# nickmccleery/open-kinematics

Measured on AMD Instinct MI355X. Metric: constraint solves/sec (sweep steps/sec), double-wishbone bump sweep, higher is better.
Workload: dtype f64

## Files before the change

### __graft_entry__.py

```python

from __future__ import annotations

import os
import sys

REPO = os.path.dirname(os.path.abspath(__file__))
if REPO not in sys.path:
    sys.path.insert(0, REPO)


def build() -> None:
    os.environ.setdefault("PYTORCH_ROCM_ARCH", "gfx950")
    from open_kinematics_amd import _lib

    path = _lib.build()
    if not os.path.exists(path):
        raise RuntimeError("libokx.so was not produced")
    from oracle import oracle as oracle_mod

    oracle_mod.build()
    import open_kinematics_amd

    lib = _lib.load()
    missing = [name for name in _lib.EXPORTS + _lib.DEBUG_EXPORTS if not hasattr(lib, name)]
# ... 8 lines not shown

def precompile_baseline_kernels() -> None:
    from open_kinematics_amd import _lib
    from open_kinematics_amd._abi import HostProgram
    from open_kinematics_amd.workloads import axle_grid_problem, bump_sweep_problem, macpherson_grid_problem

    lib = _lib.load()
    programs = []
    evaluated = []
    for make in (bump_sweep_problem, lambda n, line_mode: macpherson_grid_problem(n, n, line_mode),
                 lambda n, line_mode: axle_grid_problem(n, n, line_mode)):
        for mode in ("pinned", "softnorm"):
            programs.append(make(4, line_mode=mode)[0])
    from open_kinematics_amd.input import load_geometry, load_sweep
    from open_kinematics_amd.metrics import corner_roles
    from open_kinematics_amd.solver import dropin_program
    from open_kinematics_amd.sweep import sweep_program
    from open_kinematics_amd.workloads import geometry_path

    for geometry, sweeps in (("geometry.yaml", ("bump_sweep.yaml", "sweep.yaml")),
                             ("axle_geometry_rocker.yaml", ("axle_rocker_sweep.yaml",)),
                             ("axle_geometry.yaml", ("axle_sweep.yaml",)),
                             ("axle_geometry_explicit.yaml", ("axle_sweep.yaml",)),
                             ("macpherson_axle_geometry.yaml", ("axle_sweep.yaml",)),
                             ("corner_rocker_geometry.yaml", ("sweep.yaml",)),
                             ("corner_strut_geometry.yaml", ("sweep.yaml",)),
                             ("corner_strut_rocker_geometry.yaml", ("sweep.yaml",))):
        suspension = load_geometry(geometry_path(geometry))
        for sweep_file in sweeps:
            sweep = load_sweep(geometry_path(sweep_file), suspension)
            programs.append(dropin_program(suspension.initial_state(), suspension.constraints(), sweep,
                                           suspension.derived_spec())[0])
            programs.append(sweep_program(suspension, sweep)[0])
            if not hasattr(suspension, "corners"):
                evaluated += [(p, corner_roles(suspension, p)) for p in programs[-2:]]
            else:
                evaluated += _axle_evaluated(suspension, programs[-2:])
    evaluated.append((bump_sweep_problem(4)[0], corner_roles(load_geometry(geometry_path("geometry.yaml")), bump_sweep_problem(4)[0])))
    evaluated.append((macpherson_grid_problem(4, 4)[0],
                      corner_roles(load_geometry(geometry_path("macpherson_geometry.yaml")), macpherson_grid_problem(4, 4)[0])))
    evaluated += _axle_evaluated(load_geometry(geometry_path("axle_geometry_rocker.yaml")), [axle_grid_problem(4, 4)[0]])
    import glob

    import numpy as np

    from open_kinematics_amd.program import ConstraintProgram

    golden = os.path.join(os.path.dirname(os.path.abspath(__file__)), "tests", "golden")
    for path in sorted(glob.glob(os.path.join(golden, "[ctue]*.npz"))):
        arrays = dict(np.load(path, allow_pickle=False))
        if "prog_point_kind" not in arrays and not any(k.startswith("prog_") for k in arrays):
            continue
        fixture = ConstraintProgram.from_arrays(arrays, prefix="prog_")
        programs += [fixture.with_line_mode("pinned"), fixture]
    import yaml

    from open_kinematics_amd.input import build_suspension, build_sweep

    for path in sorted(glob.glob(os.path.join(golden, "[cte]*.npz"))):
        arrays = dict(np.load(path, allow_pickle=False))
        if "geometry_yaml" not in arrays or "sweep_yaml" not in arrays:
            continue
        try:
            suspension = build_suspension(yaml.safe_load(str(arrays["geometry_yaml"])))
            sweep = build_sweep(yaml.safe_load(str(arrays["sweep_yaml"])), suspension)
            pair = [dropin_program(suspension.initial_state(), suspension.constraints(), sweep, suspension.derived_spec())[0],
                    sweep_program(suspension, sweep)[0]]
        except Exception as error:
            print(f"precompile: drop-in programs of {os.path.basename(path)} skipped ({type(error).__name__}: {error})", file=sys.stderr)
            continue
        programs += pair
        if not hasattr(suspension, "corners"):
            evaluated += [(p, corner_roles(suspension, p)) for p in pair]
        else:
            evaluated += _axle_evaluated(suspension, pair)
    from open_kinematics_amd.metrics import roles_from_arrays

    for name in ("c1_dw_corner", "c4_macpherson_grid", "e2e_sweep"):
        arrays = dict(np.load(os.path.join(golden, f"{name}.npz"), allow_pickle=False))
        fixture = ConstraintProgram.from_arrays(arrays, prefix="prog_").with_line_mode("pinned")
        names = [fixture.point_keys[k].lower_name for k in fixture.out_point]
        metric_arrays = dict(np.load(os.path.join(golden, f"metrics_{name}.npz"), allow_pickle=False))
        evaluated.append((fixture, roles_from_arrays(names, fixture.design_pos[fixture.out_point], metric_arrays)[0]))
    from open_kinematics_amd.precompile import precompile_job

    seen, jobs = set(), []
    for program, roles in [(p, None) for p in programs] + evaluated:
        arrays = program.to_arrays()
        key = (program.line_mode, tuple((k, v.tobytes()) for k, v in sorted(arrays.items()) if k != "target_desc"),
               None if roles is None else bytes(roles))
        if key not in seen:
            seen.add(key)
            jobs.append((arrays, program.line_mode, None if roles is None else bytes(roles)))
    workers = max(1, min(6, (os.cpu_count() or 2) - 1, len(jobs)))
    try:
        results = _precompile_in_workers(jobs, workers)
    except OSError as error:
        print(f"precompile: worker pool unavailable ({type(error).__name__}: {error}); compiling sequentially", file=sys.stderr)
        results = [precompile_job(job) for job in jobs]
    for rc, message in results:
        if rc == -2:
            continue
        if rc != 0:
            raise RuntimeError(f"quad kernel precompilation failed: {message}")


def _precompile_in_workers(jobs: list, workers: int) -> list:
    import json
    import pickle
    import selectors
    import subprocess
    import tempfile

    results = [None] * len(jobs)
    pending = list(range(len(jobs)))[::-1]
    env = dict(os.environ, PYTHONPATH=os.pathsep.join([REPO] + [p for p in [os.environ.get("PYTHONPATH")] if p]))
    with tempfile.TemporaryDirectory() as tmp:
        path = os.path.join(tmp, "jobs.pkl")
        with open(path, "wb") as fh:
            pickle.dump(jobs, fh)
        procs = [subprocess.Popen([sys.executable, "-m", "open_kinematics_amd.precompile", "--jobs", path], cwd=REPO, env=env,
                                  stdin=subprocess.PIPE, stdout=subprocess.PIPE, text=True) for _ in range(workers)]
        selector = selectors.DefaultSelector()

        def feed(proc) -> bool:
            if not pending:
                proc.stdin.close()
                return False
            proc.stdin.write(f"{pending.pop()}\n")
            proc.stdin.flush()
            return True

        try:
            for proc in procs:
                if feed(proc):
                    selector.register(proc.stdout, selectors.EVENT_READ, proc)
            while selector.get_map():
                for key, _ in selector.select():
                    line = key.fileobj.readline()
                    if not line:
                        raise RuntimeError(f"a precompile worker exited with status {key.data.wait()}")
                    index, rc, message = json.loads(line)
                    results[index] = (rc, message)
                    if not feed(key.data):
                        selector.unregister(key.fileobj)
        finally:
            for proc in procs:
                if proc.poll() is None and not proc.stdin.closed:
                    proc.stdin.close()
            for proc in procs:
                proc.wait()
    return results


def _axle_evaluated(axle, programs) -> list:
    from open_kinematics_amd.metrics import axle_evaluation_roles

    out = []
    for program in programs:
        try:
            out.append((program, axle_evaluation_roles(axle, program)[0]))
        except ValueError as error:
            print(f"precompile: axle evaluated module skipped ({error})", file=sys.stderr)
    return out


def smoke() -> None:
    import numpy as np
    import torch

    from open_kinematics_amd.batch import DeviceProgram
    from open_kinematics_amd.workloads import bump_sweep_problem
    from oracle.oracle import Oracle

    if not torch.cuda.is_available():
        raise RuntimeError("smoke() needs cuda:0")
    torch.cuda.set_device(0)
    program, targets = bump_sweep_problem(101)
    dp = DeviceProgram(program, "cuda:0")
    res = dp.solve(torch.as_tensor(targets, device="cuda:0"))
    torch.cuda.synchronize()
    info = res.info()
    if not np.all((info["flags"] & 7) == 1):
        raise RuntimeError(f"smoke: not every step converged: flags={np.unique(info['flags'])}")
    orc = Oracle(program).sweep(targets, 1e-15, 1e-15, 1e-15, warm_start=False)
    err = float(np.max(np.abs(res.positions.cpu().numpy() - orc.positions)))
    if not err <= 1e-9:
        raise RuntimeError(f"smoke: device vs oracle max |dpos| = {err:.3e} mm > 1e-9")
    print(f"smoke ok: 101 steps, max|device - oracle| = {err:.2e} mm, "
          f"iterations mean {info['iterations'].mean():.2f}")


if __name__ == "__main__":
    build()
    if len(sys.argv) > 1 and sys.argv[1] == "smoke":
        smoke()
```

### open_kinematics_amd/csrc/okx_quadgen.cpp

```cpp
#include <cstdarg>
#include <cstdio>
#include <cstdlib>
#include <functional>
#include <map>
#include <set>
#include <string>
#include <vector>

#include "okx_gen.hpp"
#include "okx_plan.hpp"
#include "okx_quad.hpp"

namespace okx {
namespace {

struct LV {
  std::string n;
  int sg = 1;
};

struct Blk {
  bool scaled = true;
  std::string s;
  std::string col[3];
};

struct BlkTerm {
  Blk b;
  int sg;
};

class Gen : public GenBase {
 public:
  explicit Gen(const DevProgram& prog, const PairView* pair = nullptr)
      : GenBase(prog, pair && pair->joins.size() == 1 ? pair->couple_point : -1), pv(pair) {}

  const PairView* pv;

  static std::string sel(int i0, int i1) {
    if (i0 == i1) return std::to_string(i0);
    return "(q1 ? " + std::to_string(i1) + " : " + std::to_string(i0) + ")";
  }
  std::string point3(int p) const {
    return pv ? sel(3 * pv->pt[0][p], 3 * pv->pt[1][p]) : std::to_string(3 * p);
  }
  std::string point4(int p) const {
    return pv ? sel(4 * pv->pt[0][p], 4 * pv->pt[1][p]) : std::to_string(4 * p);
  }
  std::string crow8(int i, int k) const {
    return pv ? sel(8 * pv->row[0][i] + k, 8 * pv->row[1][i] + k) : std::to_string(8 * i + k);
  }
  std::string trow8(int i, int k) const {
    if (!pv) return std::to_string(8 * i + k);
    const int t = target_of_row(i);
    int t0 = pv->tgt[0][t], t1 = pv->tgt[1][t];
    if (t0 < 0) t0 = t1;
    if (t1 < 0) t1 = t0;
    return sel(8 * (pv->n_prog_crows + t0) + k, 8 * (pv->n_prog_crows + t1) + k);
  }
  std::string target_slot(int t) const {
    if (!pv) return std::to_string(t);
    int t0 = pv->tgt[0][t], t1 = pv->tgt[1][t];
    if (t0 < 0) t0 = t1;
    if (t1 < 0) t1 = t0;
    return sel(t0, t1);
  }
  std::string target_enable(int t) const {
    if (!pv) return "1.0";
    const bool e0 = pv->tgt[0][t] >= 0, e1 = pv->tgt[1][t] >= 0;
    if (e0 && e1) return "1.0";
    return e0 ? "(q1 ? 0.0 : 1.0)" : "(q1 ? 1.0 : 0.0)";
  }
  std::string dop_slot(int e) const { return pv ? sel(pv->dop[0][e], pv->dop[1][e]) : std::to_string(e); }
  std::map<std::string, std::string> rot1_, rot2_;
  std::map<std::string, std::vector<std::string>> bc_;
  std::map<int, std::map<int, Blk>> dblk;
  bool nz[kMaxFree][kMaxFree] = {};

  static std::string f_str(const char* fmt, ...) {
    char buf[256];
    va_list ap;
    va_start(ap, fmt);
// ... 245 lines not shown
            nb.scaled = false;
            apply_t(col, nb.col);
            acc[kv.first].push_back({nb, sg});
          }
        }
        dblk[e] = combine(acc);
      }
      return true;
    }
    why = "unknown derived op";
    return false;
  }

  struct RowOut {
    std::string r;
    std::vector<std::pair<int, LV>> partial;
    std::string absres;
  };

  std::string dp(int e) {
    auto key = std::make_pair(-1 - e, 0);
    auto it = hoisted_names.find(key);
    if (it != hoisted_names.end()) return it->second;
    char name[48], line[200];
    std::snprintf(name, sizeof(name), "hd%d", e);
    const std::string home = scalar_home(name);
    std::snprintf(line, sizeof(line), "      %s%s = a.dop_param[%s];\n", sdecl(), home.c_str(), dop_slot(e).c_str());
    hoisted += line;
    hoisted_names[key] = home;
    return home;
  }

  std::string rp(int i, int k) {
    i = pin_leader(i);
    auto key = std::make_pair(i, 100 + k);
    auto it = hoisted_names.find(key);
    if (it != hoisted_names.end()) return it->second;
    char name[48], line[200];
    std::snprintf(name, sizeof(name), "hs%d_%d", i, k);
    const std::string home = scalar_home(name);
    if (i < P.n_crows)
      std::snprintf(line, sizeof(line), "      %s%s = gq[%s];\n", sdecl(), home.c_str(), crow8(i, k).c_str());
    else
      std::snprintf(line, sizeof(line), "      %s%s = a.row_param[%s];\n", sdecl(), home.c_str(), trow8(i, k).c_str());
    hoisted += line;
    hoisted_names[key] = home;
    return home;
  }
  std::string hoisted;
  std::map<std::pair<int, int>, std::string> hoisted_names;
  bool lds_constants = false;

  int n_scalar_slots = 0, n_lane_slots = 0;
  bool scalars_in_regs = false, lanes_in_regs = false;
  std::string scalar_home(const char* name) {
    if (!lds_constants || scalars_in_regs) return name;
    return "hsl[" + std::to_string(16 * n_scalar_slots++) + " + qs]";
  }
  std::string lane_home(const char* name) {
    if (!lds_constants || lanes_in_regs) return name;
    return "hql[" + std::to_string(64 * n_lane_slots++) + " + lane]";
  }
  const char* sdecl() const { return lds_constants && !scalars_in_regs ? "" : "const double "; }
  const char* ldecl() const { return lds_constants && !lanes_in_regs ? "" : "const double "; }
  std::string rpv(int i, int k0) {
    i = pin_leader(i);
    auto key = std::make_pair(i, k0);
    auto it = hoisted_names.find(key);
    if (it != hoisted_names.end()) return it->second;
    char name[48], line[200];
    std::snprintf(name, sizeof(name), "hq%d_%d", i, k0);
    const std::string home = lane_home(name);
    if (i < P.n_crows)
      std::snprintf(line, sizeof(line), "      %s%s = ld3(gq + %s + cc, c);\n", ldecl(), home.c_str(), crow8(i, k0).c_str());
    else
      std::snprintf(line, sizeof(line), "      %s%s = ld3(a.row_param + %s + cc, c) * %s;\n", ldecl(), home.c_str(),
                    trow8(i, k0).c_str(), target_enable(target_of_row(i)).c_str());
    hoisted += line;
    hoisted_names[key] = home;
    return home;
  }
  std::map<int, std::string> pin_cross_;

  bool row(int i, RowOut* ro) {
    const int type = P.row_type[i];
    const int* pts = P.row_pts[i];
    f("    // row %d (type %d)", i, type);
    std::string r = "r" + std::to_string(i);
    ro->r = r;
    ro->absres = "fabs(" + r + ")";
    switch (type) {
      case OKX_ROW_DISTANCE:
      case OKX_ROW_SPHERICAL: {
        std::string d = vsub(pn(pts[1]), pn(pts[0]));
        std::string s = dot(d, d);
        std::string root = tmp("rt"), inv = tmp("iv"), g = tmp("g");
        f("    double %s, %s; fast_sqrt_rsqrt(%s + EPS_SQ, &%s, &%s);", root.c_str(), inv.c_str(), s.c_str(),
          root.c_str(), inv.c_str());
        f("    const double %s = %s * %s;", g.c_str(), d.c_str(), inv.c_str());
        if (type == OKX_ROW_DISTANCE)
          f("    const double %s = (%s - EPS) - %s;", r.c_str(), root.c_str(), rp(i, 0).c_str());
        else
          f("    const double %s = %s - EPS;", r.c_str(), root.c_str());
        ro->partial.push_back({pts[0], {g, -1}});
        ro->partial.push_back({pts[1], {g, 1}});
        return true;
      }
      case OKX_ROW_ANGLE:
      case OKX_ROW_THREE_POINT_ANGLE: {
        std::string v1, v2;
        if (type == OKX_ROW_ANGLE) {
          v1 = vsub(pn(pts[1]), pn(pts[0]));
          v2 = vsub(pn(pts[3]), pn(pts[2]));
        } else {
          v1 = vsub(pn(pts[0]), pn(pts[1]));
          v2 = vsub(pn(pts[2]), pn(pts[1]));
        }
        std::string cv = cross(v1, v2);
        std::string c2 = dot(cv, cv);
        std::string dt = dot(v1, v2);
        std::string s = tmp("s"), is = tmp("is"), t15 = tmp("t");
        f("    const double %s = EPS_SQ + %s;", t15.c_str(), c2.c_str());
        f("    double %s, %s; fast_sqrt_rsqrt(%s, &%s, &%s);", s.c_str(), is.c_str(), t15.c_str(), s.c_str(),
          is.c_str());
        std::string inv = tmp("iv"), ka = tmp("ka"), kb = tmp("kb");
        f("    const double %s = fast_rcp(%s + %s * %s);", inv.c_str(), t15.c_str(), dt.c_str(), dt.c_str());
        f("    const double %s = %s * %s * %s, %s = %s * %s;", ka.c_str(), dt.c_str(), inv.c_str(), is.c_str(),
          kb.c_str(), s.c_str(), inv.c_str());
        std::string w1 = cross(v2, cv), w2 = cross(cv, v1);
        std::string g1 = tmp("g"), g2 = tmp("g");
        f("    const double %s = %s * %s - %s * %s;", g1.c_str(), ka.c_str(), w1.c_str(), kb.c_str(), v2.c_str());
        f("    const double %s = %s * %s - %s * %s;", g2.c_str(), ka.c_str(), w2.c_str(), kb.c_str(), v1.c_str());
        f("    const double %s = lean_atan2_pos<%s>(%s - EPS, %s, %s) - %s;", r.c_str(), pv ? "true" : "false", s.c_str(), dt.c_str(), pv ? "atl" : "nullptr",
          rp(i, 0).c_str());
        if (type == OKX_ROW_ANGLE) {
          ro->partial.push_back({pts[0], {g1, -1}});
          ro->partial.push_back({pts[1], {g1, 1}});
          ro->partial.push_back({pts[2], {g2, -1}});
          ro->partial.push_back({pts[3], {g2, 1}});
        } else {
          std::string gm = tmp("g");
          f("    const double %s = -%s - %s;", gm.c_str(), g1.c_str(), g2.c_str());
          ro->partial.push_back({pts[0], {g1, 1}});
          ro->partial.push_back({pts[1], {gm, 1}});
          ro->partial.push_back({pts[2], {g2, 1}});
        }
        return true;
      }
      case OKX_ROW_VECTORS_PARALLEL:
      case OKX_ROW_VECTORS_PERPENDICULAR: {
        std::string v1 = vsub(pn(pts[1]), pn(pts[0])), v2 = vsub(pn(pts[3]), pn(pts[2]));
        std::string n1 = dot(v1, v1), n2 = dot(v2, v2);
        std::string s1 = tmp("s"), s2 = tmp("s"), g1 = tmp("g"), g2 = tmp("g");
        f("    const double %s = sqrt(EPS_SQ + %s), %s = sqrt(EPS_SQ + %s);", s1.c_str(), n1.c_str(), s2.c_str(), n2.c_str());
        if (type == OKX_ROW_VECTORS_PARALLEL) {
          std::string cv = cross(v1, v2);
          std::string c2 = dot(cv, cv);
          std::string sc = tmp("s");
          f("    const double %s = sqrt(EPS_SQ + %s);", sc.c_str(), c2.c_str());
          std::string w1 = cross(v2, cv), w2 = cross(cv, v1);
          std::string k26 = tmp("k"), k19 = tmp("k"), k31 = tmp("k");
          f("    const double %s = 1.0 / (%s * %s * %s), %s = %s / (%s * %s * %s * %s), %s = %s / (%s * %s * %s * %s);",
            k26.c_str(), s1.c_str(), s2.c_str(), sc.c_str(), k19.c_str(), sc.c_str(), s2.c_str(), s1.c_str(), s1.c_str(),
            s1.c_str(), k31.c_str(), sc.c_str(), s1.c_str(), s2.c_str(), s2.c_str(), s2.c_str());
          f("    const double %s = %s * %s - %s * %s, %s = %s * %s - %s * %s;", g1.c_str(), k26.c_str(), w1.c_str(),
            k19.c_str(), v1.c_str(), g2.c_str(), k26.c_str(), w2.c_str(), k31.c_str(), v2.c_str());
          f("    const double %s = (%s - EPS) / ((%s - EPS) * (%s - EPS));", r.c_str(), sc.c_str(), s1.c_str(), s2.c_str());
        } else {
          std::string dt = dot(v1, v2);
          std::string k16 = tmp("k"), k18 = tmp("k"), k19 = tmp("k");
          f("    const double %s = 1.0 / (%s * %s), %s = %s / (%s * %s * %s * %s), %s = %s / (%s * %s * %s * %s);",
            k16.c_str(), s1.c_str(), s2.c_str(), k18.c_str(), dt.c_str(), s2.c_str(), s1.c_str(), s1.c_str(), s1.c_str(),
            k19.c_str(), dt.c_str(), s1.c_str(), s2.c_str(), s2.c_str(), s2.c_str());
          f("    const double %s = %s * %s - %s * %s, %s = %s * %s - %s * %s;", g1.c_str(), k16.c_str(), v2.c_str(),
            k18.c_str(), v1.c_str(), g2.c_str(), k16.c_str(), v1.c_str(), k19.c_str(), v2.c_str());
          f("    const double %s = %s / ((%s - EPS) * (%s - EPS));", r.c_str(), dt.c_str(), s1.c_str(), s2.c_str());
        }
        ro->partial.push_back({pts[0], {g1, -1}});
        ro->partial.push_back({pts[1], {g1, 1}});
        ro->partial.push_back({pts[2], {g2, -1}});
        ro->partial.push_back({pts[3], {g2, 1}});
        return true;
      }
      case OKX_ROW_EQUAL_DISTANCE: {
        std::string d1 = vsub(pn(pts[1]), pn(pts[0])), d2 = vsub(pn(pts[3]), pn(pts[2]));
        std::string s1 = dot(d1, d1), s2 = dot(d2, d2);
        std::string r1 = tmp("rt"), i1 = tmp("iv"), r2 = tmp("rt"), i2 = tmp("iv");
        f("    double %s, %s, %s, %s; fast_sqrt_rsqrt(%s + EPS_SQ, &%s, &%s); fast_sqrt_rsqrt(%s + EPS_SQ, &%s, &%s);",
          r1.c_str(), i1.c_str(), r2.c_str(), i2.c_str(), s1.c_str(), r1.c_str(), i1.c_str(), s2.c_str(),
          r2.c_str(), i2.c_str());
        std::string g1 = tmp("g"), g2 = tmp("g");
        f("    const double %s = %s * %s, %s = %s * %s;", g1.c_str(), d1.c_str(), i1.c_str(), g2.c_str(), d2.c_str(),
          i2.c_str());
        f("    const double %s = (%s - EPS) - (%s - EPS);", r.c_str(), r1.c_str(), r2.c_str());
        ro->partial.push_back({pts[0], {g1, -1}});
        ro->partial.push_back({pts[1], {g1, 1}});
        ro->partial.push_back({pts[2], {g2, 1}});
        ro->partial.push_back({pts[3], {g2, -1}});
        return true;
      }
      case OKX_ROW_FIXED_AXIS: {
        const int ax = (int)P.row_param[i][0];
        std::string pa = bcast(pn(pts[0]), ax);
        f("    const double %s = %s - %s;", r.c_str(), pa.c_str(), rp(i, 1).c_str());
        ro->partial.push_back({pts[0], {"e" + std::to_string(ax), 1}});
        return true;
      }
// ... 24 lines not shown
        const int comp = (int)P.row_param[i][6];
        std::string g = cross(ld, "e" + std::to_string(comp));
        std::string rc = bcast(cv, comp);
        f("    const double %s = %s;", r.c_str(), rc.c_str());
        ro->partial.push_back({pts[0], {g, 1}});
        if (comp == 0) {
          std::string c2 = dot(cv, cv);
          ro->absres = "fabs(lean_sqrt(" + c2 + " + EPS_SQ) - EPS)";
        } else {
          ro->absres.clear();
        }
        return true;
      }
      case OKX_ROW_POINT_ON_PLANE: {
        std::string pp = rpv(i, 0), nn = rpv(i, 3);
        std::string w = vsub(pn(pts[0]), pp);
        std::string d = dot(w, nn);
        f("    const double %s = %s;", r.c_str(), d.c_str());
        ro->partial.push_back({pts[0], {nn, 1}});
        return true;
      }
      case OKX_ROW_MIDPOINT_ON_PLANE: {
        std::string pp = rpv(i, 0), nn = rpv(i, 3);
        std::string mid = tmp("m");
        f("    const double %s = %s + (%s - %s) * 0.5;", mid.c_str(), pn(pts[0]).c_str(), pn(pts[1]).c_str(),
          pn(pts[0]).c_str());
        std::string w = vsub(mid, pp);
        std::string d = dot(w, nn);
        std::string h = tmp("h");
        f("    const double %s = 0.5 * %s;", h.c_str(), nn.c_str());
        f("    const double %s = %s;", r.c_str(), d.c_str());
        ro->partial.push_back({pts[0], {h, 1}});
        ro->partial.push_back({pts[1], {h, 1}});
        return true;
      }
      case OKX_ROW_COPLANAR:
      case OKX_ROW_SCALAR_TRIPLE: {
        std::string v1 = vsub(pn(pts[1]), pn(pts[0])), v2 = vsub(pn(pts[2]), pn(pts[0])),
                    v3 = vsub(pn(pts[3]), pn(pts[0]));
        std::string c23 = cross(v2, v3), c31 = cross(v3, v1), c12 = cross(v1, v2);
        std::string vol = dot(v1, c23);
        std::string g1 = c23, g2 = c31, g3 = c12;
        if (type == OKX_ROW_SCALAR_TRIPLE) {
          std::string isc = tmp("is");
          f("    const double %s = fast_rcp(%s);", isc.c_str(), rp(i, 1).c_str());
          g1 = tmp("g"), g2 = tmp("g"), g3 = tmp("g");
          f("    const double %s = %s * %s, %s = %s * %s, %s = %s * %s;", g1.c_str(), c23.c_str(), isc.c_str(),
            g2.c_str(), c31.c_str(), isc.c_str(), g3.c_str(), c12.c_str(), isc.c_str());
          f("    const double %s = (%s - %s) * %s;", r.c_str(), vol.c_str(), rp(i, 0).c_str(), isc.c_str());
        } else {
          f("    const double %s = %s;", r.c_str(), vol.c_str());
        }
        std::string g0 = tmp("g");
        f("    const double %s = -(%s + %s + %s);", g0.c_str(), g1.c_str(), g2.c_str(), g3.c_str());
        ro->partial.push_back({pts[0], {g0, 1}});
        ro->partial.push_back({pts[1], {g1, 1}});
        ro->partial.push_back({pts[2], {g2, 1}});
        ro->partial.push_back({pts[3], {g3, 1}});
        return true;
      }
      case kRowTarget: {
        std::string dir = rpv(i, 0);
        std::string d = dot(pn(pts[0]), dir);
        f("    const double %s = %s - %s * tv%d;", r.c_str(), d.c_str(), target_enable(target_of_row(i)).c_str(),
          target_of_row(i));
        ro->partial.push_back({pts[0], {dir, 1}});
        return true;
      }
      default:
        why = "row type " + std::to_string(type) + " has no quad code path yet";
        return false;
    }
  }

  static std::string A(int F, int G, int k) {
    return "A" + std::to_string(F) + "_" + std::to_string(G) + "_" + std::to_string(k);
  }
  static std::string Ln(int F, int G, int k) {
    return "L" + std::to_string(F) + "_" + std::to_string(G) + "_" + std::to_string(k);
  }

  bool emit_rows_residual_only() {
    f("    double ss = 0.0, mres_new = 0.0;");
    for (int i = 0; i < P.m; ++i) {
      RowOut ro;
      if (!row(i, &ro)) return false;
      f("    ss = fma(%s, %s, ss);", ro.r.c_str(), ro.r.c_str());
      if (!ro.absres.empty()) f("    mres_new = fmax(mres_new, %s);", ro.absres.c_str());
    }
    return true;
  }

  bool pin_ata = false, pin_atr = false;
  bool marks = false;
  bool tl_marks = false;
  void mark(int n) {
    if (marks) f("    __builtin_amdgcn_sched_barrier(0); asm volatile(\"s_nop %d\"); __builtin_amdgcn_sched_barrier(0);", 10 + n);
    if (tl_marks && n >= 5) f("    OKX_TL(%d)", n);
  }
  std::vector<std::string> jtv_rhs;
  std::function<std::string(int, int)> jtv_value;
  bool jtv_only = true;
  bool emit_rows() {
    const int nf = P.n_free;
    const bool jtv = !jtv_rhs.empty() && jtv_only;
    for (int F = 0; F < nf; ++F) {
      for (const std::string& q : jtv_rhs) f("    double %sg%d = 0.0;", q.c_str(), F);
      if (!jtv) f("    double gn%d = 0.0;", F);
      nz[F][F] = true;
    }
    if (!jtv) f("    double ss = 0.0, mres_new = 0.0;");
    std::set<std::string> declared;
    for (int i = 0; i < P.m; ++i) {
      RowOut ro;
      mark(1);
      if (!row(i, &ro)) return false;
      if (!jtv) {
      f("    ss = fma(%s, %s, ss);", ro.r.c_str(), ro.r.c_str());
      if (!ro.absres.empty()) f("    mres_new = fmax(mres_new, %s);", ro.absres.c_str());
      }
      mark(2);
      std::map<int, std::vector<LV>> terms;
      for (auto& pp : ro.partial) {
        const int pt = pp.first;
        const LV& gp = pp.second;
        if (blk_of_point[pt] >= 0) {
          terms[blk_of_point[pt]].push_back(gp);
        } else if (dop_of_point[pt] >= 0) {
          auto it = dblk.find(dop_of_point[pt]);
          if (it == dblk.end()) {
            why = "row reads a derived point without chain blocks";
            return false;
          }
          for (auto& kv : it->second) {
            const Blk& b = kv.second;
            std::string t = tmp("j");
            if (b.scaled) {
              f("    const double %s = (%s) * %s;", t.c_str(), b.s.c_str(), gp.n.c_str());
            } else {
              std::string b0 = bcast(gp.n, 0), b1 = bcast(gp.n, 1), b2 = bcast(gp.n, 2);
              f("    const double %s = %s * %s + %s * %s + %s * %s;", t.c_str(), b0.c_str(), b.col[0].c_str(),
                b1.c_str(), b.col[1].c_str(), b2.c_str(), b.col[2].c_str());
            }
            terms[kv.first].push_back({t, gp.sg});
          }
        }
      }
      std::vector<std::pair<int, LV>> jv;
      for (auto& kv : terms) {
        if (kv.second.size() == 1) {
          jv.push_back({kv.first, kv.second[0]});
        } else {
          std::string e;
          for (auto& t : kv.second) {
            if (!e.empty()) e += t.sg < 0 ? " - " : " + ";
            else if (t.sg < 0) e += "-";
            e += t.n;
          }
          std::string t = tmp("j");
          f("    const double %s = %s;", t.c_str(), e.c_str());
          jv.push_back({kv.first, {t, 1}});
        }
      }
      for (size_t qi = 0; qi < jtv_rhs.size(); ++qi) {
        const std::string& q = jtv_rhs[qi];
        if (jtv_value) f("    const double %s%d = %s;", q.c_str(), i, jtv_value((int)qi, i).c_str());
        for (auto& fv : jv) f("    %sg%d = fma(%s, %s%d, %sg%d);", q.c_str(), fv.first, sx(fv.second).c_str(), q.c_str(), i, q.c_str(), fv.first);
      }
      if (jtv) continue;
      if (P.row_type[i] == kRowTarget) target_j[(int)P.row_param[i][3]] = jv;
      for (auto& fv : jv) f("    gn%d = fma(%s, %s, gn%d);", fv.first, sx(fv.second).c_str(), ro.r.c_str(), fv.first);
      if (pin_atr)
        for (auto& fv : jv) f("    asm volatile(\"\" : \"+v\"(gn%d));", fv.first);
      mark(3);
      std::vector<std::string> touched;
      for (size_t ia = 0; ia < jv.size(); ++ia)
        for (size_t ib = 0; ib <= ia; ++ib) {
          const int F = jv[ia].first, G = jv[ib].first;
          const LV& jF = jv[ia].second;
          const LV& jG = jv[ib].second;
          nz[F][G] = true;
          for (int k = 0; k < 3; ++k) {
            std::string b = bcast(jG.n, k);
            const int sg = jF.sg * jG.sg;
            std::string an = A(F, G, k);
            if (!declared.count(an)) {
              declared.insert(an);
              f("    double %s = %s%s * %s;", an.c_str(), sg < 0 ? "-" : "", jF.n.c_str(), b.c_str());
            } else {
              f("    %s = fma(%s%s, %s, %s);", an.c_str(), sg < 0 ? "-" : "", jF.n.c_str(), b.c_str(), an.c_str());
            }
            touched.push_back(an);
          }
        }
      if (pin_ata)
        for (auto& an : touched) f("    asm volatile(\"\" : \"+v\"(%s));", an.c_str());
      mark(4);
    }
// ... 578 lines not shown
    mov_index.assign(NP, -1);
    int MVN = 0;
    if (EVP)
      for (int p = 0; p < NP; ++p)
        if (used[p] && (g.blk_of_point[p] >= 0 || g.dop_of_point[p] >= 0)) mov_index[p] = MVN++;
    MV = 3 * MVN;
    out_loc.assign(prog_out, OutLoc{-1, -1});
    if (EVP)
      for (int sd = 0; sd < 2; ++sd)
        for (int k = 0; k < P.n_out; ++k)
          if (pv->out[sd][k] >= 0 && (sd == 0 || pv->out[1][k] != pv->out[0][k])) out_loc[pv->out[sd][k]] = {sd, P.out_point[k]};
    if (EVP)
      for (int t = 0; t < T; ++t)
        for (int sd = 0; sd < 2; ++sd)
          if (pv->tgt[sd][t] >= 0) ev_jobs.push_back({t, sd, pv->tgt[sd][t]});
    if (EV) {
      if (T < 1) {
        why = "an evaluated module needs at least one target";
        return false;
      }
      std::vector<int> oi(NP, -1);
      for (int k = 0; k < P.n_out; ++k) oi[P.out_point[k]] = k;
      for (int F = 0; F < nf; ++F)
        if (oi[ev.fp(F)] < 0) {
          why = "an evaluated module needs every free point among the output points";
          return false;
        }
      epi_factor_src = capture(ev, [&] { ev.emit_factor(); });
    }
    Gen fin(P, pv);
    fin.uid = 100000;
    fin.hoisted_names = ev.hoisted_names;
    for (int e = 0; e < P.n_derived; ++e)
      if (!fin.derived_op(e, false)) {
        why = fin.why;
        return false;
      }
    final_src = fin.out;
    return true;
  }
  int vel_offset(int k) const {
    const OutLoc& l = out_loc[k];
    if (l.side < 0 || mov_index[l.point] < 0) return -1;
    return l.side * MV + 3 * mov_index[l.point];
  }

  void emit_preamble_and_helpers() {
    g.out += kPreamble;
    if (EV) {
      g.out += eval_metrics_source(*es);
      if (EVP) {
        g.out += eval_roles_source();
        g.f("struct QEvArgs { QArgs q; double* tan; double* ev; EvCfg cfg; EvCfg cfg_r; EvRoleNum roles[8]; };");
        std::string table = "__constant__ short kVelMap[" + std::to_string(3 * prog_out) + "] = {";
        for (int k = 0; k < prog_out; ++k)
          for (int cc2 = 0; cc2 < 3; ++cc2) {
            const int off = vel_offset(k);
            table += (k || cc2 ? ", " : "") + std::to_string(off < 0 ? -1 : off + cc2);
          }
        g.out += table + "};  // record element -> offset in a problem-target block of the staged velocities\n";
      } else
        g.f("struct QEvArgs { QArgs q; double* tan; double* ev; EvCfg cfg; };");
      g.f("#define EV_WAVE_SYNC() do { __builtin_amdgcn_fence(__ATOMIC_RELEASE, \"wavefront\"); __builtin_amdgcn_wave_barrier(); __builtin_amdgcn_fence(__ATOMIC_ACQUIRE, \"wavefront\"); } while (0)");
    }
    if (ev.tl_marks) g.f("#define OKX_TL(k)");
    g.f("");
    if (pv) {
      g.f("// Two quads own one problem: `xq` reads the other quad's lane with the same component");
      g.f("// (ds_swizzle, lane ^ 4: data path only, no LDS memory); PSUM / PMAX reduce over both quads and");
      g.f("// are bit-identical in all eight lanes (commutative combination of the two quad results).");
      g.f("DEV double xq(double v) {");
      g.f("  int lo = __builtin_amdgcn_ds_swizzle(__double2loint(v), 0x101F);");
      g.f("  int hi = __builtin_amdgcn_ds_swizzle(__double2hiint(v), 0x101F);");
      g.f("  return __hiloint2double(hi, lo);");
      g.f("}");
      if (EVP) g.f("DEV Du<1> du_xq(Du<1> a) { Du<1> r; r.v = xq(a.v); r.d[0] = xq(a.d[0]); return r; }");
      g.f("DEV double PSUM(double v) { const double s = qsum(v); return s + xq(s); }");
      g.f("DEV double PMAX(double v) { const double s = qmax(v); return fmax(s, xq(s)); }");
      g.f("#define PJOIN_SUM(v) ((v) + xq(v))");
    } else {
      g.f("#define PSUM(v) qsum(v)");
      g.f("#define PMAX(v) qmax(v)");
      g.f("#define PJOIN_SUM(v) (v)");
    }
    g.f("");
  }

  std::string epilogue_src(const std::string& contig) {
    ev.reset_caches();
    bool ok = true;
    const std::string text = capture(ev, [&] { ok = EVP ? emit_pair_epilogue(contig) : emit_epilogue(contig); });
    ev.reset_caches();
    return ok ? text : std::string();
  }
  bool emit_epilogue(const std::string& contig) {
    ev.f("    {  // ---- evaluated epilogue: tangents at the solved state, metrics and their derivatives along them ----");
    ev.out += eval_src;
    ev.f("    const double lambda = 0.0;  // (an undamped factorisation; shadows the solve's damping)");
    declare_factor_registers(ev);
    ev.out += epi_factor_src;
    ev.f("    __shared__ __attribute__((aligned(16))) double vst[16 * %d];  // velocities [quad][target][record]", T * REC);
    for (int t = 0; t < T; ++t) {
      ev.f("    {  // target %d: (J^T J) q = J^T e_t, then the velocity of every point", t);
      std::vector<std::string> rhs(nf, "0.0");
      auto it = ev.target_j.find(t);
      if (it != ev.target_j.end())
        for (auto& fv : it->second) rhs[fv.first] = Gen::sx(fv.second);
      ev.emit_substitute(rhs, "tq");
      const std::string vp = "w" + std::to_string(t) + "_";
      for (int p = 0; p < NP; ++p) {
        if (!used[p] || ev.dop_of_point[p] >= 0) continue;
        if (ev.blk_of_point[p] >= 0) ev.f("    const double %s%d = tq%d;", vp.c_str(), p, ev.blk_of_point[p]);
        else ev.f("    const double %s%d = 0.0;", vp.c_str(), p);
      }
      for (int e = 0; e < P.n_derived; ++e)
        if (!ev.derived_jvp(e, vp)) return false;
      ev.f("    if (c < 3) {");
      ev.f("      double* vs = vst + (quad * %d + %d) * %d + c;", T, t, REC);
      for (int k = 0; k < P.n_out; ++k) ev.f("      vs[%d] = ok ? %s%d : __builtin_nan(\"\");", 3 * k, vp.c_str(), P.out_point[k]);
      ev.f("    }");
      ev.f("    }");
    }
    ev.f("    EV_WAVE_SYNC();");
    ev.f("    const long long ev_rem = a.n_problems - wu * 16;");
    ev.f("    const int ev_rows = (int)(ev_rem < 16 ? ev_rem : 16);  // problems of a contiguous wavefront block");
    auto copy_out = [&](const char* dst, const char* stage_name, int per_problem) {
      ev.f("      if (%s) {", contig.c_str());
      ev.f("        const int n_doubles = ev_rows * %d;", per_problem);
      ev.f("        double2* dst = reinterpret_cast<double2*>(%s + wu * 16 * %d);", dst, per_problem);
      ev.f("        const double2* src = reinterpret_cast<const double2*>(%s);", stage_name);
      ev.f("        for (int i = lane; i < n_doubles / 2; i += 64) dst[i] = src[i];");
      ev.f("        if ((n_doubles & 1) && lane == 0) (%s + wu * 16 * %d)[n_doubles - 1] = %s[n_doubles - 1];", dst, per_problem, stage_name);
      ev.f("      } else if (valid) {  // chains: a quad's problems are far apart in memory");
      ev.f("        double* dst = %s + bb * %d;", dst, per_problem);
      ev.f("        const double* src = %s + quad * %d;", stage_name, per_problem);
      ev.f("        for (int i = c; i < %d; i += 4) dst[i] = src[i];", per_problem);
      ev.f("      }");
    };
    ev.f("    if (ea.tan != nullptr) {");
    copy_out("ea.tan", "vst", T * REC);
    ev.f("    }");
    ev.f("    if (ea.ev != nullptr) {");
    ev.f("      __shared__ __attribute__((aligned(16))) double est[16 * %d];  // [quad][row][column]", (1 + T) * EVC);
    ev.f("      EvCfg cfg = ea.cfg;");
    ev.f("      if (PG) {  // an ensemble's design references are its geometry's own");
    ev.f("        cfg.design_wheel_center_z = gp[%d]; cfg.design_contact_patch_z = gp[%d];", 3 * P.out_point[es->wheel_center] + 2,
         3 * P.out_point[es->contact_patch] + 2);
    if (es->rack >= 0) ev.f("        cfg.design_rack_y = gp[%d];", 3 * P.out_point[es->rack] + 1);
    ev.f("      }");
    ev.f("      const double ev_flags = (ok ? 1.0 : 0.0) + ((!ok || pmin <= %d * 2.220446049250313e-16 * pmax) ? 2.0 : 0.0);", 3 * nf);
    ev.f("      _Pragma(\"unroll 1\")");
    ev.f("      for (int ep = 0; 4 * ep <= %d; ++ep) {", T);
    ev.f("        const int evt = 4 * ep + c - 1;  // this lane's direction: -1 the values, t the derivative along target t");
    ev.f("        const bool dir = evt >= 0 && evt < %d;", T);
    ev.f("        const double* ps = stage + quad * %d;", REC);
    ev.f("        const double* vs = vst + (quad * %d + (dir ? evt : 0)) * %d;", T, REC);
    ev.f("        DV<1> RP[EV_SLOTS];");
    for (int sl = 0; sl < kEvalSlots; ++sl) {
      const int k = eval_slot_point(*es, sl);
      if (k < 0) {
        ev.f("        RP[%d].x = du_const<1>(0.0); RP[%d].y = du_const<1>(0.0); RP[%d].z = du_const<1>(0.0);", sl, sl, sl);
        continue;
      }
      for (int cc2 = 0; cc2 < 3; ++cc2)
        ev.f("        RP[%d].%c.v = ps[%d]; RP[%d].%c.d[0] = dir ? vs[%d] : 0.0;", sl, "xyz"[cc2], 3 * k + cc2, sl, "xyz"[cc2], 3 * k + cc2);
    }
// ... 2067 lines not shown
```

Before: 1.022 billion.

## Batch norm chains of up to four rows across quad lanes in generated kernels

The quad kernel generator now groups distance, spherical and angle rows in sets of up to four. Their squared-norm reductions go through one transposed quad sum, so lane k holds row k's sum, followed by a single sqrt/rsqrt. Each row then broadcasts its result from lane k. This replaces up to four separate quad reductions and sqrt chains with one, cutting cross-lane shuffles and transcendental latency, at the cost of extra selects and broadcasts. The old serial path stays behind a dev switch and is also precompiled.

```diff
diff --git a/__graft_entry__.py b/__graft_entry__.py
--- a/__graft_entry__.py
+++ b/__graft_entry__.py
@@ -114,6 +114,9 @@
         names = [fixture.point_keys[k].lower_name for k in fixture.out_point]
         metric_arrays = dict(np.load(os.path.join(golden, f"metrics_{name}.npz"), allow_pickle=False))
         evaluated.append((fixture, roles_from_arrays(names, fixture.design_pos[fixture.out_point], metric_arrays)[0]))
+    arrays = dict(np.load(os.path.join(golden, "rows_all_classes.npz"), allow_pickle=False))
+    all_classes = ConstraintProgram.from_arrays(arrays, prefix="prog_")
+    programs.append(all_classes)
     from open_kinematics_amd.precompile import precompile_job
 
     seen, jobs = set(), []
@@ -130,6 +133,23 @@
     except OSError as error:
         print(f"precompile: worker pool unavailable ({type(error).__name__}: {error}); compiling sequentially", file=sys.stderr)
         results = [precompile_job(job) for job in jobs]
+    serial = [bump_sweep_problem(4)[0], macpherson_grid_problem(4, 4)[0], axle_grid_problem(4, 4)[0]]
+    for name in ("c1_dw_corner", "t_corner_strut_rocker", "t_corner_rocker"):
+        arrays = dict(np.load(os.path.join(golden, f"{name}.npz"), allow_pickle=False))
+        serial.append(ConstraintProgram.from_arrays(arrays, prefix="prog_").with_line_mode("pinned"))
+    serial.append(all_classes)
+    serial_jobs = [(p.to_arrays(), p.line_mode, None) for p in serial]
+    try:
+        results += _precompile_in_workers(serial_jobs, max(1, min(workers, len(serial_jobs))), dev="quad_serial_chains")
+    except OSError:
+        kept = os.environ.get("OKX_DEV")
+        os.environ["OKX_DEV"] = "quad_serial_chains"
+        try:
+            results += [precompile_job(job) for job in serial_jobs]
+        finally:
+            os.environ.pop("OKX_DEV")
+            if kept is not None:
+                os.environ["OKX_DEV"] = kept
     for rc, message in results:
         if rc == -2:
             continue
@@ -137,7 +157,7 @@
             raise RuntimeError(f"quad kernel precompilation failed: {message}")
 
 
-def _precompile_in_workers(jobs: list, workers: int) -> list:
+def _precompile_in_workers(jobs: list, workers: int, dev: str | None = None) -> list:
     import json
     import pickle
     import selectors
@@ -147,6 +167,8 @@
     results = [None] * len(jobs)
     pending = list(range(len(jobs)))[::-1]
     env = dict(os.environ, PYTHONPATH=os.pathsep.join([REPO] + [p for p in [os.environ.get("PYTHONPATH")] if p]))
+    if dev is not None:
+        env["OKX_DEV"] = dev
     with tempfile.TemporaryDirectory() as tmp:
         path = os.path.join(tmp, "jobs.pkl")
         with open(path, "wb") as fh:
diff --git a/open_kinematics_amd/csrc/okx_quadgen.cpp b/open_kinematics_amd/csrc/okx_quadgen.cpp
--- a/open_kinematics_amd/csrc/okx_quadgen.cpp
+++ b/open_kinematics_amd/csrc/okx_quadgen.cpp
@@ -1,3 +1,4 @@
+#include <algorithm>
 #include <cstdarg>
 #include <cstdio>
 #include <cstdlib>
@@ -409,6 +410,58 @@
   }
   std::map<int, std::string> pin_cross_;
 
+  bool batch_chains = !dev_switch("quad_serial_chains");
+  bool batched_any = false;
+  struct ChainPre { std::string d, v1, v2, x, rt, iv, re; int lane; };
+  static bool chain_row(int type) {
+    return type == OKX_ROW_DISTANCE || type == OKX_ROW_SPHERICAL || type == OKX_ROW_ANGLE || type == OKX_ROW_THREE_POINT_ANGLE;
+  }
+  std::map<int, ChainPre> chain_pre_;
+  std::map<int, std::vector<int>> chain_batches() const {
+    std::map<int, std::vector<int>> res;
+    if (!batch_chains) return res;
+    std::vector<int> rows;
+    for (int i = 0; i < P.m; ++i)
+      if (chain_row(P.row_type[i])) rows.push_back(i);
+    for (size_t k = 0; k + 1 < rows.size(); k += 4)
+      res[rows[k]] = std::vector<int>(rows.begin() + k, rows.begin() + std::min(k + 4, rows.size()));
+    return res;
+  }
+  void emit_chain_batch(const std::vector<int>& rows) {
+    const int n = (int)rows.size();
+    std::string sq;
+    for (int k = 0; k < n; ++k) {
+      const int* pts = P.row_pts[rows[k]];
+      ChainPre& cp = chain_pre_[rows[k]];
+      cp.lane = k;
+      const int type = P.row_type[rows[k]];
+      if (type == OKX_ROW_DISTANCE || type == OKX_ROW_SPHERICAL) {
+        cp.d = vsub(pn(pts[1]), pn(pts[0]));
+      } else {
+        if (type == OKX_ROW_ANGLE) {
+          cp.v1 = vsub(pn(pts[1]), pn(pts[0]));
+          cp.v2 = vsub(pn(pts[3]), pn(pts[2]));
+        } else {
+          cp.v1 = vsub(pn(pts[0]), pn(pts[1]));
+          cp.v2 = vsub(pn(pts[2]), pn(pts[1]));
+        }
+        cp.d = cross(cp.v1, cp.v2);
+      }
+      sq += cp.d + " * " + cp.d + ", ";
+    }
+    std::string s = tmp("cs"), x = tmp("cx"), root = tmp("rt"), inv = tmp("iv"), re = tmp("re");
+    f("    // norm chains of rows %d..%d, row k in lane k", rows.front(), rows.back());
+    f("    const double %s = qsum_t%d(%sc);", s.c_str(), n, sq.c_str());
+    f("    const double %s = %s + EPS_SQ;", x.c_str(), s.c_str());
+    f("    double %s, %s; fast_sqrt_rsqrt(%s, &%s, &%s);", root.c_str(), inv.c_str(), x.c_str(), root.c_str(), inv.c_str());
+    f("    const double %s = %s - EPS;", re.c_str(), root.c_str());
+    for (int k = 0; k < n; ++k) {
+      ChainPre& cp = chain_pre_[rows[k]];
+      cp.x = x, cp.rt = root, cp.iv = inv, cp.re = re;
+    }
+    batched_any = true;
+  }
+
   bool row(int i, RowOut* ro) {
     const int type = P.row_type[i];
     const int* pts = P.row_pts[i];
@@ -419,6 +472,20 @@
     switch (type) {
       case OKX_ROW_DISTANCE:
       case OKX_ROW_SPHERICAL: {
+        auto cp = chain_pre_.find(i);
+        if (cp != chain_pre_.end()) {
+          const ChainPre& c = cp->second;
+          std::string inv = tmp("iv"), re = tmp("re"), g = tmp("g");
+          f("    const double %s = QB%d(%s), %s = QB%d(%s);", inv.c_str(), c.lane, c.iv.c_str(), re.c_str(), c.lane, c.re.c_str());
+          f("    const double %s = %s * %s;", g.c_str(), c.d.c_str(), inv.c_str());
+          if (type == OKX_ROW_DISTANCE)
+            f("    const double %s = %s - %s;", r.c_str(), re.c_str(), rp(i, 0).c_str());
+          else
+            f("    const double %s = %s;", r.c_str(), re.c_str());
+          ro->partial.push_back({pts[0], {g, -1}});
+          ro->partial.push_back({pts[1], {g, 1}});
+          return true;
+        }
         std::string d = vsub(pn(pts[1]), pn(pts[0]));
         std::string s = dot(d, d);
         std::string root = tmp("rt"), inv = tmp("iv"), g = tmp("g");
@@ -435,7 +502,17 @@
       }
       case OKX_ROW_ANGLE:
       case OKX_ROW_THREE_POINT_ANGLE: {
-        std::string v1, v2;
+        std::string v1, v2, cv, dt;
+        std::string s, is, t15;
+        auto cp = chain_pre_.find(i);
+        if (cp != chain_pre_.end()) {
+          const ChainPre& c = cp->second;
+          v1 = c.v1, v2 = c.v2, cv = c.d;
+          dt = dot(v1, v2);
+          s = tmp("s"), is = tmp("is"), t15 = tmp("t");
+          f("    const double %s = QB%d(%s), %s = QB%d(%s), %s = QB%d(%s);", t15.c_str(), c.lane, c.x.c_str(), s.c_str(), c.lane,
+            c.rt.c_str(), is.c_str(), c.lane, c.iv.c_str());
+        } else {
         if (type == OKX_ROW_ANGLE) {
           v1 = vsub(pn(pts[1]), pn(pts[0]));
           v2 = vsub(pn(pts[3]), pn(pts[2]));
@@ -443,13 +520,14 @@
           v1 = vsub(pn(pts[0]), pn(pts[1]));
           v2 = vsub(pn(pts[2]), pn(pts[1]));
         }
-        std::string cv = cross(v1, v2);
+        cv = cross(v1, v2);
         std::string c2 = dot(cv, cv);
-        std::string dt = dot(v1, v2);
-        std::string s = tmp("s"), is = tmp("is"), t15 = tmp("t");
+        dt = dot(v1, v2);
+        s = tmp("s"), is = tmp("is"), t15 = tmp("t");
         f("    const double %s = EPS_SQ + %s;", t15.c_str(), c2.c_str());
         f("    double %s, %s; fast_sqrt_rsqrt(%s, &%s, &%s);", s.c_str(), is.c_str(), t15.c_str(), s.c_str(),
           is.c_str());
+        }
         std::string inv = tmp("iv"), ka = tmp("ka"), kb = tmp("kb");
         f("    const double %s = fast_rcp(%s + %s * %s);", inv.c_str(), t15.c_str(), dt.c_str(), dt.c_str());
         f("    const double %s = %s * %s * %s, %s = %s * %s;", ka.c_str(), dt.c_str(), inv.c_str(), is.c_str(),
@@ -640,8 +718,10 @@
 
   bool emit_rows_residual_only() {
     f("    double ss = 0.0, mres_new = 0.0;");
+    const std::map<int, std::vector<int>> batches = chain_batches();
     for (int i = 0; i < P.m; ++i) {
       RowOut ro;
+      if (batches.count(i)) emit_chain_batch(batches.at(i));
       if (!row(i, &ro)) return false;
       f("    ss = fma(%s, %s, ss);", ro.r.c_str(), ro.r.c_str());
       if (!ro.absres.empty()) f("    mres_new = fmax(mres_new, %s);", ro.absres.c_str());
@@ -669,9 +749,11 @@
     }
     if (!jtv) f("    double ss = 0.0, mres_new = 0.0;");
     std::set<std::string> declared;
+    const std::map<int, std::vector<int>> batches = chain_batches();
     for (int i = 0; i < P.m; ++i) {
       RowOut ro;
       mark(1);
+      if (batches.count(i)) emit_chain_batch(batches.at(i));
       if (!row(i, &ro)) return false;
       if (!jtv) {
       f("    ss = fma(%s, %s, ss);", ro.r.c_str(), ro.r.c_str());
@@ -1416,6 +1498,32 @@
       g.f("#define PSUM(v) qsum(v)");
       g.f("#define PMAX(v) qmax(v)");
       g.f("#define PJOIN_SUM(v) (v)");
+    }
+    if (ev.batched_any) {
+      g.f("// Transposed quad sums (batched norm chains): lane k of the quad gets the quad sum of s<k>, in qsum's association");
+      g.f("// (s[k] + s[k^1]) + (s[k^2] + s[k^3]) - bit for bit what qsum(s<k>) gives.  Round one exchanges with lane ^ 1 (even");
+      g.f("// lanes keep s0 / s2, odd lanes s1 / s3), round two with lane ^ 2.  For sums of squares only (no signed zeros).");
+      g.f("#define QB3(v) qperm<0xFF>(v)");
+      g.f("DEV double qsum_t2(double s0, double s1, int c) {");
+      g.f("#pragma clang fp contract(off)");
+      g.f("  const bool odd = (c & 1) != 0;");
+      g.f("  const double a = (odd ? s1 : s0) + qperm<0xB1>(odd ? s0 : s1);");
+      g.f("  return a + qperm<0x4E>(a);");
+      g.f("}");
+      g.f("DEV double qsum_t3(double s0, double s1, double s2, int c) {");
+      g.f("#pragma clang fp contract(off)");
+      g.f("  const bool odd = (c & 1) != 0, hi = (c & 2) != 0;");
+      g.f("  const double a = (odd ? s1 : s0) + qperm<0xB1>(odd ? s0 : s1);");
+      g.f("  const double b = s2 + qperm<0xB1>(s2);");
+      g.f("  return (hi ? b : a) + qperm<0x4E>(hi ? a : b);");
+      g.f("}");
+      g.f("DEV double qsum_t4(double s0, double s1, double s2, double s3, int c) {");
+      g.f("#pragma clang fp contract(off)");
+      g.f("  const bool odd = (c & 1) != 0, hi = (c & 2) != 0;");
+      g.f("  const double a = (odd ? s1 : s0) + qperm<0xB1>(odd ? s0 : s1);");
+      g.f("  const double b = (odd ? s3 : s2) + qperm<0xB1>(odd ? s2 : s3);");
+      g.f("  return (hi ? b : a) + qperm<0x4E>(hi ? a : b);");
+      g.f("}");
     }
     g.f("");
   }
```

After: 1.054 billion, median of 6. 1.03x the previous value.
